# oneapi-src/ishmem

Hardware: AMD Instinct MI355X
Metric: GiB/s device-resident float32 sum-reduce at 1/2/4/8 PEs vs HBM+xGMI roofline (higher is better)
Workload: dtype f32

## Files before the change

include/ishmem_capi.h:

```cpp
#ifndef ISHMEM_AMD_CAPI_H
#define ISHMEM_AMD_CAPI_H

#include <stddef.h>
#include <stdint.h>

#ifdef __cplusplus
extern "C" {
#endif

typedef enum {
    ISHMEMI_OP_AND = 0,
    ISHMEMI_OP_OR = 1,
    ISHMEMI_OP_XOR = 2,
    ISHMEMI_OP_MAX = 3,
    ISHMEMI_OP_MIN = 4,
    ISHMEMI_OP_SUM = 5,
    ISHMEMI_OP_PROD = 6,
    ISHMEMI_OP_COUNT = 7
} ishmemi_c_op_t;

typedef enum {
    ISHMEMI_DT_INT8 = 0,
    ISHMEMI_DT_INT16 = 1,
    ISHMEMI_DT_INT32 = 2,
// ... 99 lines not shown
int ishmemi_c_fence(void);
int ishmemi_c_quiet_on_stream(void *stream);
int ishmemi_c_read_all_u32(void *out, const void *p, size_t n, int grid, void *stream);

#define ISHMEMI_C_MAX_PES 16
#define ISHMEMI_C_MAX_TEAMS 64
#define ISHMEMI_C_DEV_PHASES 4
typedef struct {
    int32_t pe, npes;
    uint64_t timeout_ticks;
    char *heap_base;
    uint64_t heap_size;
    char *peer_heap[ISHMEMI_C_MAX_PES];
    uint32_t *my_dflags;
    uint32_t *peer_dflags[ISHMEMI_C_MAX_PES];
    uint32_t *epochs;
    uint32_t *err;
    int32_t team_start[ISHMEMI_C_MAX_TEAMS], team_stride[ISHMEMI_C_MAX_TEAMS];
    int32_t team_size[ISHMEMI_C_MAX_TEAMS], team_my_idx[ISHMEMI_C_MAX_TEAMS];
    uint64_t *dev_counts;
} ishmemi_c_device_ctx_t;
void *ishmemi_c_device_ctx(void);
int ishmemi_c_register_device_ctx_slot(const void *host_shadow);

const char *ishmemi_c_last_error(void);
int ishmemi_c_set_param(const char *name, long long value);
long long ishmemi_c_get_param(const char *name);
int ishmemi_c_phase_times(float *ms5);
int ishmemi_c_error_count(void);
size_t ishmemi_c_dtype_size(int dtype);
int ishmemi_c_op_dtype_valid(int op, int dtype);
int ishmemi_c_chunk_bounds(uint64_t nitems, int npes, int c, uint64_t *begin, uint64_t *end);
int ishmemi_c_path_limits(int npes, int colocated, long long *ll_limit, long long *fold_limit);
int ishmemi_c_bootstrap_selftest(int pe, int npes, const char *key, int value, int *out);
const char *ishmemi_c_version(void);

#ifdef __cplusplus
}
#endif

#endif
```

ishmem_amd/_lib.py:

```python
from __future__ import annotations

import ctypes
import os
from pathlib import Path

LIB_PATH = Path(__file__).resolve().parent / "libishmem_amd.so"
_VARIANT = os.environ.get("ISHMEM_AMD_LIB")

_vp, _i, _sz, _ll, _u64 = ctypes.c_void_p, ctypes.c_int, ctypes.c_size_t, ctypes.c_longlong, ctypes.c_uint64
PROTOTYPES = [
    ("ishmemi_c_init", _i, []),
    ("ishmemi_c_init_pe", _i, [_i, _i, _i, ctypes.c_char_p]),
    ("ishmemi_c_launch_info", _i, [ctypes.POINTER(_i), ctypes.POINTER(_i), ctypes.POINTER(_i), ctypes.c_char_p, _sz,
                                   ctypes.c_char_p, _sz]),
    ("ishmemi_c_finalize", _i, []),
    ("ishmemi_c_initialized", _i, []),
    ("ishmemi_c_my_pe", _i, []),
    ("ishmemi_c_n_pes", _i, []),
    ("ishmemi_c_device", _i, []),
    ("ishmemi_c_init_thread", _i, [_i, ctypes.POINTER(_i)]),
    ("ishmemi_c_query_thread", _i, [ctypes.POINTER(_i)]),
    ("ishmemi_c_malloc", _vp, [_sz]),
    ("ishmemi_c_align", _vp, [_sz, _sz]),
    ("ishmemi_c_calloc", _vp, [_sz, _sz]),
# ... 23 lines not shown
    ("ishmemi_c_fcollect", _i, [_i, _vp, _vp, _sz]),
    ("ishmemi_c_fcollect_on_stream", _i, [_i, _vp, _vp, _sz, _vp, _vp]),
    ("ishmemi_c_alltoall", _i, [_i, _vp, _vp, _sz]),
    ("ishmemi_c_alltoall_on_stream", _i, [_i, _vp, _vp, _sz, _vp, _vp]),
    ("ishmemi_c_collect_on_stream", _i, [_i, _vp, _vp, _sz, _vp, _vp]),
    ("ishmemi_c_put", _i, [_vp, _vp, _sz, _i]),
    ("ishmemi_c_get", _i, [_vp, _vp, _sz, _i]),
    ("ishmemi_c_put_nbi", _i, [_vp, _vp, _sz, _i]),
    ("ishmemi_c_get_nbi", _i, [_vp, _vp, _sz, _i]),
    ("ishmemi_c_put_on_stream", _i, [_vp, _vp, _sz, _i, _vp]),
    ("ishmemi_c_get_on_stream", _i, [_vp, _vp, _sz, _i, _vp]),
    ("ishmemi_c_quiet", _i, []),
    ("ishmemi_c_fence", _i, []),
    ("ishmemi_c_quiet_on_stream", _i, [_vp]),
    ("ishmemi_c_read_all_u32", _i, [_vp, _vp, _sz, _i, _vp]),
    ("ishmemi_c_stream_wait_events", _i, [_vp, _vp, _sz]),
    ("ishmemi_c_stream_record_event", _i, [_vp, _vp]),
    ("ishmemi_c_collect", _i, [_i, _vp, _vp, _sz]),
    ("ishmemi_c_scan", _i, [_i, _i, _i, _vp, _vp, _sz]),
    ("ishmemi_c_scan_on_stream", _i, [_i, _i, _i, _vp, _vp, _sz, _vp, _vp]),
    ("ishmemi_c_broadcast", _i, [_i, _vp, _vp, _sz, _i]),
    ("ishmemi_c_broadcast_on_stream", _i, [_i, _vp, _vp, _sz, _i, _vp, _vp]),
    ("ishmemi_c_device_ctx", _vp, []),
    ("ishmemi_c_register_device_ctx_slot", _i, [_vp]),
    ("ishmemi_c_last_error", ctypes.c_char_p, []),
    ("ishmemi_c_set_param", _i, [ctypes.c_char_p, _ll]),
    ("ishmemi_c_get_param", _ll, [ctypes.c_char_p]),
    ("ishmemi_c_phase_times", _i, [ctypes.POINTER(ctypes.c_float)]),
    ("ishmemi_c_error_count", _i, []),
    ("ishmemi_c_dtype_size", _sz, [_i]),
    ("ishmemi_c_op_dtype_valid", _i, [_i, _i]),
    ("ishmemi_c_chunk_bounds", _i, [_u64, _i, _i, ctypes.POINTER(_u64), ctypes.POINTER(_u64)]),
    ("ishmemi_c_path_limits", _i, [_i, _i, ctypes.POINTER(_ll), ctypes.POINTER(_ll)]),
    ("ishmemi_c_bootstrap_selftest", _i, [_i, _i, ctypes.c_char_p, _i, ctypes.POINTER(_i)]),
    ("ishmemi_c_version", ctypes.c_char_p, []),
]

_lib = None


def load(build_if_missing: bool = True) -> ctypes.CDLL:
    global _lib
    if _lib is not None:
        return _lib
    if _VARIANT:
        lib = ctypes.CDLL(str(Path(_VARIANT).resolve()), mode=ctypes.RTLD_GLOBAL)
        for name, res, args in PROTOTYPES:
            fn = getattr(lib, name)
            fn.restype = res
            fn.argtypes = args
        _lib = lib
        return lib
    if build_if_missing:
        from . import _build
        if _build.needs_build():
            try:
                _build.build()
            except RuntimeError:
                if not LIB_PATH.exists():
                    raise
    if not LIB_PATH.exists():
        raise ImportError(f"ishmem_amd native library missing: {LIB_PATH} (run __graft_entry__.build())")
    lib = ctypes.CDLL(str(LIB_PATH), mode=ctypes.RTLD_GLOBAL)
    for name, res, args in PROTOTYPES:
        fn = getattr(lib, name)
        fn.restype = res
        fn.argtypes = args
    _lib = lib
    _warn_foreign_runtime()
    return lib


def _warn_foreign_runtime() -> None:
    try:
        with open("/proc/self/maps") as f:
            foreign = any("amdhip64" in line and "/torch/lib/" in line for line in f)
    except OSError:
        return
    if foreign:
        import sys
        print("[ishmem_amd] WARN: the HIP runtime in use is torch's bundled copy (torch was imported "
# ... 3 lines not shown
```

ishmem_amd/csrc/kernels.h:

```cpp
#pragma once
#include <hip/hip_runtime.h>
#include <stddef.h>
#include <stdint.h>

#include "types.h"

namespace ishmemi {

constexpr int kMaxPes = 16;
constexpr int kMaxBlocks = 1024;
constexpr int kPhases = 4;
constexpr int kPhaseStart = 0, kPhaseMid = 1, kPhaseEnd = 2, kPhaseSync = 3;
constexpr size_t kFlagWordsPerTeam = (size_t) kPhases * kMaxBlocks * kMaxPes;
constexpr size_t kTeamFlagBytes = kFlagWordsPerTeam * 4 + 256;
constexpr int kBlock = 256;
constexpr int kUnroll = 4;
constexpr int kFaninBlock = 64;
constexpr int kFaninMaxGrid = (int) ((1ull << 31) / kFaninBlock);

constexpr int kEpWords = 16;
constexpr int kLineWords = 16;
constexpr int kEpReplicas = 64;
constexpr int kEpRepLine = 1, kEpShardLine = kEpRepLine + kEpReplicas, kEpShards = 8;
constexpr int kEpTopLine = kEpShardLine + kEpShards;
// ... 109 lines not shown
constexpr int kRealignMaxGrid = (int) ((1ull << 31) / kRealignBlock);
#ifndef ISHMEMI_RS_REALIGN_BLOCK
#define ISHMEMI_RS_REALIGN_BLOCK 64
#endif
constexpr int kRsRealignBlock = ISHMEMI_RS_REALIGN_BLOCK;
#ifndef ISHMEMI_REALIGN_PEEL
#define ISHMEMI_REALIGN_PEEL 256
#endif
constexpr uint64_t kRealignPeel = ISHMEMI_REALIGN_PEEL;

struct FaninArgs {
    const char *src[kMaxFanin];
    char *dst;
    uint64_t head, nitems, tail;
    int nsrc;
    int realign;
    uint32_t shift[kMaxFanin];
    uint64_t total;
};

struct PhaseArgs {
    const char *src[kMaxPes];
    const char *dstp[kMaxPes];
    char *dst;
    uint64_t head, nitems, tail;
    uint64_t items_per_chunk;
    uint32_t elem;
    int p, me;
    int peer_nt;
    uint32_t shift;
    uint64_t total;
    int whole;
    int xcd_group;
};
hipError_t launch_rs_phase(int op, int dt, const PhaseArgs &a, hipStream_t s);
hipError_t launch_ag_phase(const PhaseArgs &a, hipStream_t s);

hipError_t launch_allreduce(int op, int dt, bool vec, const ReduceArgs &a, int grid,
                            hipStream_t s);
hipError_t launch_fanin(int op, int dt, bool vec, const FaninArgs &a, int grid, hipStream_t s);
hipError_t launch_team_sync(const ReduceArgs &a, hipStream_t s);
hipError_t launch_pull_probe(const FaninArgs &a, int policy, hipStream_t s);
void set_device_share(int share);
int device_share();
constexpr int kWaitSlotsDefault = 16;
void set_wait_slots(int slots);
int wait_slots();
void set_realign_grid_cap(int cap);
int realign_grid_cap();
void set_collect_realign(int on);
int collect_realign();
void set_phase_unaligned(int on);
int phase_unaligned();
hipError_t launch_occupy(int grid, uint64_t usec, hipStream_t s);
hipError_t launch_produce_u32(uint32_t *dst, const uint32_t *a, const uint32_t *b, uint64_t n, hipStream_t s);

struct RmaArgs {
    char *dst;
    const char *src;
    uint64_t head, nitems, tail;
};
hipError_t launch_rma_copy(const RmaArgs &a, bool put, int max_blocks, hipStream_t s);
hipError_t launch_read_all_u32(uint32_t *out, const uint32_t *p, uint64_t n, int grid, hipStream_t s);

}
```

ishmem_amd/csrc/kernels.hip:

```cpp
#include "kernels_impl.h"

namespace ishmemi {

namespace {
int g_device_share = 1;
int g_wait_slots = kWaitSlotsDefault;
}
void set_device_share(int share) { g_device_share = share < 1 ? 1 : share; }
int device_share() { return g_device_share; }
void set_wait_slots(int slots) { g_wait_slots = slots < 1 ? 1 : slots; }
int wait_slots() { return g_wait_slots; }
int g_realign_grid_cap = 0;
void set_realign_grid_cap(int cap) { g_realign_grid_cap = cap < 0 ? 0 : cap; }
int realign_grid_cap() { return g_realign_grid_cap; }
int g_collect_realign = 1;
void set_collect_realign(int on) { g_collect_realign = on != 0; }
int collect_realign() { return g_collect_realign; }
int g_phase_unaligned = 1;
void set_phase_unaligned(int on) { g_phase_unaligned = on != 0; }
int phase_unaligned() { return g_phase_unaligned; }

#define ISHMEMI_DECL_OP(N)                                                                         \
    hipError_t launch_allreduce_op##N(int dt, bool vec, const ReduceArgs &a, int grid,             \
                                      hipStream_t s);                                              \
    hipError_t launch_fanin_op##N(int dt, bool vec, const FaninArgs &a, int grid, hipStream_t s); \
    hipError_t launch_ll_op##N(int dt, const LLArgs &a, hipStream_t s);                            \
    hipError_t launch_rs_phase_op##N(int dt, const PhaseArgs &a, hipStream_t s);
ISHMEMI_DECL_OP(0)
ISHMEMI_DECL_OP(1)
ISHMEMI_DECL_OP(2)
ISHMEMI_DECL_OP(3)
ISHMEMI_DECL_OP(4)
ISHMEMI_DECL_OP(5)
ISHMEMI_DECL_OP(6)

hipError_t launch_allreduce(int op, int dt, bool vec, const ReduceArgs &a, int grid, hipStream_t s)
{
    if (!op_dtype_valid(op, dt)) return hipErrorInvalidValue;
    switch (op) {
        case 0: return launch_allreduce_op0(dt, vec, a, grid, s);
        case 1: return launch_allreduce_op1(dt, vec, a, grid, s);
        case 2: return launch_allreduce_op2(dt, vec, a, grid, s);
        case 3: return launch_allreduce_op3(dt, vec, a, grid, s);
        case 4: return launch_allreduce_op4(dt, vec, a, grid, s);
        case 5: return launch_allreduce_op5(dt, vec, a, grid, s);
        case 6: return launch_allreduce_op6(dt, vec, a, grid, s);
        default: return hipErrorInvalidValue;
// ... 64 lines not shown
```

ishmem_amd/csrc/kernels_impl.h:

```cpp
#pragma once
#include <algorithm>
#include <map>
#include <mutex>
#include <type_traits>

#include "kernels.h"

namespace ishmemi {
namespace {

constexpr int kSysCoherent = 17;
constexpr int kNonTemporal = 2;
constexpr uint64_t kTile = (uint64_t) kBlock * kUnroll;
#ifndef ISHMEMI_AR_OCC
#define ISHMEMI_AR_OCC 4
#endif


template <typename T>
struct alignas(16) Vec {
    T e[16 / sizeof(T)];
};

template <typename T>
// ... 786 lines not shown
    if (i0 + tid < a.nitems) wt_store(make_rsrc(uniform_ptr(a.dst + wo)), tid * 16u, acc);
}

template <typename T, int OP, int NS>
__global__ __launch_bounds__(kRealignBlock) void fanin_realign_kernel(FaninArgs a)
{
    static_assert(NS == 1 || NS == 2, "realigned fan-in: 1 or 2 sources");
    __shared__ u32x4 edge[NS][kRealignWaves + 1];
    const uint32_t tid = threadIdx.x;
    const uint64_t stride = (uint64_t) gridDim.x * kRealignBlock;
    const uint64_t first = (uint64_t) blockIdx.x * kRealignBlock;
    if (stride >= a.nitems) {
        if (first < a.nitems) fanin_realign_block<T, OP, NS>(a, edge, first);
    } else {
        for (uint64_t i0 = first; i0 < a.nitems; i0 += stride) {
            fanin_realign_block<T, OP, NS>(a, edge, i0);
            __syncthreads();
        }
    }
    if (blockIdx.x == 0) {
        const uint64_t tail_off = a.head + a.nitems * (16 / sizeof(T));
        for (int pass = 0; pass < 2; ++pass) {
            const uint64_t cnt = pass == 0 ? a.head : a.tail;
            for (uint64_t t = tid; t < cnt; t += kRealignBlock) {
                const uint64_t e = pass == 0 ? t : tail_off + t;
                T acc = ((const T *) a.src[0])[e];
                if constexpr (NS == 2) acc = op1<T, OP>(acc, ((const T *) a.src[1])[e]);
                ((T *) a.dst)[e] = acc;
            }
        }
    }
}

template <typename T, int OP, int P, bool NT, int R>
__device__ __forceinline__ void rs_phase_item(const PhaseArgs &a, uint64_t wb, bool valid)
{
    using Item = Vec<T>;
    const uint32_t off = threadIdx.x * 16u;
    Item x[P];
#pragma unroll
    for (int k = 0; k < P; ++k) {
        const int j = (R + k) % P;
        if (!valid) continue;
        if (NT || j == a.me) x[k] = bload<Item>(make_rsrc(uniform_ptr(a.src[j] + wb)), off);
        else x[k] = cload<Item>(make_rsrc(uniform_ptr(a.src[j] + wb)), off);
    }
    Item acc = x[(P - R) % P];
#pragma unroll
    for (int j = 1; j < P; ++j) acc = op1<T, OP>(acc, x[(j - R + P) % P]);
    if (valid) wt_store(make_rsrc(uniform_ptr(a.dst + wb)), off, acc);
}

template <typename T, int OP, int P, bool NT, int R = 0>
__device__ __forceinline__ void rs_phase_dispatch(const PhaseArgs &a, int rot, uint64_t wb, bool valid)
{
    if constexpr (R == P - 1) {
        rs_phase_item<T, OP, P, NT, R>(a, wb, valid);
    } else {
        if (rot == R) rs_phase_item<T, OP, P, NT, R>(a, wb, valid);
        else rs_phase_dispatch<T, OP, P, NT, R + 1>(a, rot, wb, valid);
    }
}

template <typename T, int OP>
__device__ __forceinline__ void rs_phase_item_any(const PhaseArgs &a, uint64_t wb, bool valid)
{
    using Item = Vec<T>;
    if (!valid) return;
    const uint32_t off = threadIdx.x * 16u;
    Item acc;
    for (int j = 0; j < a.p; ++j) {
        Item x;
        if (j == a.me || a.peer_nt) x = nt_load((const Item *) (a.src[j] + wb + off));
        else x = cload<Item>(make_rsrc(uniform_ptr(a.src[j] + wb)), off);
        acc = j == 0 ? x : op1<T, OP>(acc, x);
    }
    wt_store(make_rsrc(uniform_ptr(a.dst + wb)), off, acc);
}

template <typename T, int OP>
__device__ __forceinline__ void rs_phase_edges(const PhaseArgs &a)
{
    const int p = a.p, me = a.me;
    if (blockIdx.x == 0) {
        const int tid = threadIdx.x;
        const uint64_t tail_off = a.head + a.nitems * (16 / sizeof(T));
        for (int region = 0; region < 2; ++region) {
            const bool owner = a.whole || (region == 0 ? me == 0 : me == p - 1);
            const uint64_t cnt = region == 0 ? a.head : a.tail;
            if (!owner || (uint64_t) tid >= cnt) continue;
            const uint64_t rbase = (region == 0 ? 0 : tail_off) * sizeof(T);
            const uint32_t off = (uint32_t) (tid * sizeof(T));
            T acc = T();
            for (int j = 0; j < p; ++j) {
                T x;
                if (j == me) x = ((const T *) (a.src[j] + rbase))[tid];
                else x = cload<T>(make_rsrc(uniform_ptr(a.src[j] + rbase)), off);
                acc = (j == 0) ? x : op1<T, OP>(acc, x);
            }
            wt_store(make_rsrc(uniform_ptr(a.dst + rbase)), off, acc);
        }
    }
}

__device__ __forceinline__ uint64_t xcd_grouped_block(uint64_t b, uint64_t grid)
{
    if (b >= (grid & ~63ull)) return b;
    return (b & ~63ull) | ((b & 7) << 3) | ((b >> 3) & 7);
}

template <typename T, int OP, int P>
__global__ __launch_bounds__(kFaninBlock) void rs_phase_kernel(PhaseArgs a)
{
    const int me = a.me;
    const uint64_t cs = a.whole ? 0 : min((uint64_t) me * a.items_per_chunk, a.nitems);
    const uint64_t ce = a.whole ? a.nitems : min(cs + a.items_per_chunk, a.nitems);
    const uint64_t head_bytes = a.head * sizeof(T);
    const uint64_t stride = (uint64_t) gridDim.x * kFaninBlock;
    const uint64_t blk = a.shift && a.xcd_group ? xcd_grouped_block(blockIdx.x, gridDim.x) : blockIdx.x;
    auto body = [&](auto nt) {
        for (uint64_t i0 = cs + blk * kFaninBlock; i0 < ce; i0 += stride) {
            const bool valid = i0 + threadIdx.x < ce;
            const uint64_t wb = head_bytes + i0 * 16;
            if constexpr (P > 0) rs_phase_dispatch<T, OP, P, decltype(nt)::value>(a, (int) ((i0 / kFaninBlock) % P), wb, valid);
            else rs_phase_item_any<T, OP>(a, wb, valid);
        }
    };
    if (a.peer_nt) {
        body(std::true_type{});
    } else {
        body(std::false_type{});
    }
    rs_phase_edges<T, OP>(a);
// ... 62 lines not shown
        const uint64_t je = min(js + a.items_per_chunk, a.nitems);
        const uint64_t i0 = js + (w / peers) * kFaninBlock;
        if (i0 + threadIdx.x < je) {
            const uint64_t wb = head_bytes + i0 * 16;
            const u32x4 x = a.peer_nt ? nt_load((const u32x4 *) (a.dstp[j] + wb + off))
                                      : cload<u32x4>(make_rsrc(uniform_ptr(a.dstp[j] + wb)), off);
            wt_store(make_rsrc(uniform_ptr(a.dst + wb)), off, x);
        }
    }
    if (blockIdx.x == 0) {
        const uint32_t tid = threadIdx.x;
        const uint64_t tail_b = (uint64_t) a.tail * a.elem;
        const uint64_t tail_base = head_bytes + a.nitems * 16;
        if (me != 0 && tid < head_bytes)
            a.dst[tid] = (char) cload<uint8_t>(make_rsrc(uniform_ptr(a.dstp[0])), tid);
        if (me != p - 1 && tid < tail_b)
            a.dst[tail_base + tid] = (char) cload<uint8_t>(make_rsrc(uniform_ptr(a.dstp[p - 1] + tail_base)), tid);
    }
}

template <typename K>
int phase_grid(K, uint64_t items)
{
    const uint64_t g = (items + kFaninBlock - 1) / kFaninBlock;
    return (int) std::max<uint64_t>(1, std::min<uint64_t>(g, (uint64_t) kFaninMaxGrid));
}

template <typename T, int OP>
hipError_t rs_phase_t(const PhaseArgs &a, hipStream_t s)
{
    const uint64_t cs = a.whole ? 0 : std::min((uint64_t) a.me * a.items_per_chunk, a.nitems);
    const uint64_t len = a.whole ? a.nitems : std::min(cs + a.items_per_chunk, a.nitems) - cs;
    auto go = [&](auto kernel) {
        hipLaunchKernelGGL(kernel, dim3(phase_grid(kernel, len)), dim3(kFaninBlock), 0, s, a);
    };
    if (a.shift && !phase_unaligned()) {
        uint64_t g = std::max<uint64_t>(1, std::min<uint64_t>((len + kRsRealignBlock - 1) / kRsRealignBlock,
                                                              (1ull << 31) / kRsRealignBlock));
        if (realign_grid_cap() > 0) g = std::min<uint64_t>(g, (uint64_t) realign_grid_cap());
        hipLaunchKernelGGL((rs_phase_realign_kernel<T, OP>), dim3((unsigned) g), dim3(kRsRealignBlock), 0, s, a);
    } else if (a.p == 2) go(rs_phase_kernel<T, OP, 2>);
    else if (a.p == 4) go(rs_phase_kernel<T, OP, 4>);
    else if (a.p == 8) go(rs_phase_kernel<T, OP, 8>);
    else go(rs_phase_kernel<T, OP, 0>);
    return hipGetLastError();
}

template <typename T, int OP>
__device__ __forceinline__ uint64_t fold8(uint64_t acc, uint64_t x)
{
    constexpr int K = 8 / sizeof(T);
    struct alignas(8) W {
        T e[K];
    };
    W a = __builtin_bit_cast(W, acc), b = __builtin_bit_cast(W, x);
#pragma unroll
    for (int i = 0; i < K; ++i) a.e[i] = op1<T, OP>(a.e[i], b.e[i]);
    return __builtin_bit_cast(uint64_t, a);
}

__device__ __forceinline__ uint64_t ll_load(const char *p, uint64_t valid)
{
    if (valid == 8) {
        if (((uintptr_t) p & 7) == 0) return *(const uint64_t *) p;
        if (((uintptr_t) p & 3) == 0)
            return (uint64_t) ((const uint32_t *) p)[0] | ((uint64_t) ((const uint32_t *) p)[1] << 32);
    }
// ... 230 lines not shown
```

ishmem_amd/csrc/runtime.cpp:

```cpp
#include <hip/hip_runtime.h>
#include <stdio.h>
#include <stdlib.h>
#include <string.h>
#include <strings.h>
#include <stdint.h>
#include <errno.h>
#include <sys/prctl.h>
#include <unistd.h>

#include <algorithm>
#include <chrono>
#include <limits>
#include <map>
#include <mutex>
#include <string>
#include <vector>

#include "bootstrap.h"
#include "kernels.h"
#include "types.h"

namespace ishmemi {
namespace {

// ... 134 lines not shown
    const char *b = s;
    while (*b == ' ' || *b == '\t') ++b;
    char *end = nullptr;
    errno = 0;
    const long long v = strtoll(b, &end, 10);
    const char *e = end;
    while (*e == ' ' || *e == '\t') ++e;
    if (end == b || *e || errno == ERANGE) {
        if (strncmp(name, "ISHMEM_", 7) == 0 && g_env_error.empty())
            g_env_error = std::string(name) + "='" + s + "' is not an integer";
        return dflt;
    }
    return v;
}

bool env_flag_false(const char *name)
{
    const char *s = getenv(name);
    return s && *s && (strcmp(s, "0") == 0 || strcasecmp(s, "false") == 0);
}
bool env_flag_true(const char *name)
{
    const char *s = getenv(name);
    return s && *s && !env_flag_false(name);
}

void warn_unknown_env()
{
    static const char *const known[] = {
        "DEBUG", "ENABLE_VERBOSE_PRINT", "STACK_PRINT_LIMIT", "ENABLE_GPU_IPC", "ENABLE_GPU_IPC_PIDFD",
        "SYMMETRIC_SIZE", "ENABLE_ACCESSIBLE_HOST_HEAP", "NBI_COUNT", "MWAIT_BURST", "SHMEM_LIB_NAME",
        "MPI_LIB_NAME", "PMI_LIB_NAME", "TEAMS_MAX", "TEAM_SHARED_ONLY_SELF", "RUNTIME", "RUNTIME_USE_OSHMPI", "ROOT",
        "PE", "NPES", "DEVICE", "BOOTSTRAP_KEY", "TIMEOUT_MS", "MAX_BLOCKS", "WAIT_SLOTS", "LL_MAX_BYTES",
        "ONESHOT_P2_MAX_BYTES", "PHASED_MIN_BYTES", "PHASED_PEER_NT", "STAGING_SIZE", "STAGING_SLOTS",
        "STAGED_COPY_KERNEL", "STREAM_ORDER", "FLAGS_KIND", "EP_UNCACHED", "BARRIER_KIND", "XGMI_LL_MAX_BYTES",
        "XGMI_FOLD_MAX_BYTES", "TEST_FLAGS_UNAVAILABLE", "TEST_PCI_BUS",
        "AMD_LIB", "OFFLOAD_ARCH", "BENCH_SAME_DEVICE", "BENCH_EMULATE_SHARE1", "BENCH_SETUP_WATCHDOG_S"};
    for (char **e = ::environ; e && *e; ++e) {
        if (strncmp(*e, "ISHMEM_", 7) != 0) continue;
        const char *name = *e + 7, *eq = strchr(name, '=');
        const size_t len = eq ? (size_t) (eq - name) : strlen(name);
        bool ok = false;
        for (const char *k : known) ok = ok || (strlen(k) == len && strncmp(k, name, len) == 0);
        if (!ok) fprintf(stderr, "[ishmem_amd] WARN: Environment variable 'ISHMEM_%.*s' is not a supported variable\n", (int) len, name);
    }
}

long long wait_slots_floor() { return std::max<long long>(1, env_ll("GPU_MAX_HW_QUEUES", 4)); }

struct Team {
    bool valid = false;
    int start = 0, stride = 1, size = 1;
    int my_idx = -1;
    int num_contexts = 0;
    bool colocated = true;
};

struct TeamMem {
    uint32_t *flags[kMaxPes] = {};
    uint64_t *ring[kMaxPes] = {};
    int pool_idx = -1;
    char *fold_scratch = nullptr;
    size_t fold_scratch_bytes = 0;
};

struct PoolBlock {
    uint32_t *ptr = nullptr;
    hipIpcMemHandle_t handle{};
    bool in_use = false;
};

constexpr long long kPhasedOff = std::numeric_limits<long long>::max();
constexpr long long kPhasedDefault = 4ll << 20;

struct PeRecord {
    int32_t pe, pid, device, flags_kind;
    int32_t flags_kind_requested;
    char pci_bus[32];
    uint64_t heap_size;
    int64_t max_blocks, ll_max_bytes, oneshot_p2, phased_min;
    uint64_t staging_bytes;
    int64_t staging_slots;
    int64_t xgmi_ll_max, xgmi_fold_max;
    hipIpcMemHandle_t heap_handle;
    hipIpcMemHandle_t flags_handle;
};

struct State {
    std::mutex mu;
    bool initialized = false;
    int pe = 0, npes = 1, device = 0;
    ShmBootstrap boot;

    char *heap = nullptr;
    size_t heap_size = 0;
    std::map<size_t, size_t> free_list;
    std::map<size_t, size_t> used;
    char *peer_heap[kMaxPes] = {};

    uint32_t *flags = nullptr;
    int flags_kind = 0;
    uint32_t *peer_flags[kMaxPes] = {};
    int dev_id[kMaxPes] = {};
    TeamMem tmem[kMaxTeams];
    int teams_max = kTeamsMaxDefault;
    size_t team_block_bytes = 0;
    std::vector<PoolBlock> team_pool;
    std::map<std::pair<int, uint32_t>, void *> peer_pool;
    uint32_t *err_host = nullptr;
    uint32_t *err_dev = nullptr;
    uint64_t *exch_host = nullptr, *exch_dev = nullptr;
    uint32_t *done_host = nullptr, *done_dev = nullptr;
    uint32_t done_seq = 0;
    int block_spin = 2;
    ishmemi_c_device_ctx_t *dctx = nullptr;
    uint32_t *dev_epochs = nullptr;
    uint32_t *kern_ep = nullptr;

    char *team_scratch = nullptr;
    char *count_slots = nullptr;
    char *staging = nullptr;
    size_t staging_bytes = 0;
    hipStream_t copy_in = nullptr, copy_out = nullptr;
    hipStream_t rma_stream = nullptr;
    hipEvent_t rma_ev = nullptr;
    bool rma_pending = false;
    hipStream_t last_stream = nullptr;
    bool last_stream_set = false;
    bool stream_order = false;
    long long oneshot_p2 = 32ll << 20;
    long long phased_min = kPhasedDefault;
    hipEvent_t order_ev = nullptr;
    hipEvent_t staging_ev = nullptr;
    bool staging_used = false;
    int staging_slots = kStagingSlotsDefault;
    int staged_copy_kernel = 0;
    bool test_flags_unavailable = false;
    int phased_peer_nt = 0;
    int ar_shifted = 1;
    int rs_xcd = 1;
    int direct_p2 = 1;
    int direct_max_pes = 4;
    int direct_inplace = 1;
    long long xgmi_ll_max = -1, xgmi_fold_max = -1;
    double xgmi_link_bps = 76.8e9;
    hipEvent_t ev_in[kMaxStagingSlots] = {}, ev_red[kMaxStagingSlots] = {}, ev_out[kMaxStagingSlots] = {};

    Team teams[kMaxTeams];
    int max_blocks = kMaxBlocks;
    long long ll_max_bytes = (long long) kLLDefaultBytes;
    long long timeout_ms = 60000;
    int debug = 0;
    int error_count = 0;
    uint64_t *trace = nullptr;
    bool phase_events = false, phase_recorded = false;
    hipEvent_t phase_ev[6] = {};
    double init_us[8] = {};
};

const char *const kInitPhase[8] = {"hip", "heap", "flags", "bootstrap", "ipc_heap", "ipc_flags", "teams", "total"};

State &S()
{
    static State s;
    return s;
}

struct CtxSlots {
    std::mutex mu;
    std::vector<const void *> shadows;
};
// ... 244 lines not shown
    if (f.a_us > g.a_us) return 0;
    if (f.b_us_per_byte <= g.b_us_per_byte) return kUnlimited;
    return (long long) ((g.a_us - f.a_us) / (f.b_us_per_byte - g.b_us_per_byte));
}

struct PathLimits {
    long long ll, fold, oneshot;
};

PathLimits path_limits(const State &s, int p, bool colocated)
{
    PathLimits r{0, 0, 0};
    if (p < 2) return r;
    const long long cap = std::min<long long>(std::max<long long>(s.ll_max_bytes, 0), (long long) ll_capacity(p));
    const bool fold_team = s.direct_p2 && p <= s.direct_max_pes;
    if (colocated) {
        r.ll = cap;
        if (p >= 3 && fold_team) r.ll = std::min<long long>(r.ll, (768ll << 10) / p);
        r.fold = p == 2 ? s.oneshot_p2 : s.oneshot_p2 / 4 / (p - 1);
    } else {
        const double L = s.xgmi_link_bps;
        long long ll = crossover(model_ll(p, L), model_rsag(p, L));
        if (fold_team) ll = std::min(ll, crossover(model_ll(p, L), model_fold(p, L)));
        if (s.xgmi_ll_max >= 0) ll = s.xgmi_ll_max;
        r.ll = std::min(cap, ll);
        r.fold = s.xgmi_fold_max >= 0 ? s.xgmi_fold_max : crossover(model_fold(p, L), model_rsag(p, L));
    }
    r.oneshot = r.fold;
    if (!fold_team) r.fold = 0;
    return r;
}

PathLimits team_limits(const State &s, const Team &t) { return path_limits(s, t.size, t.colocated); }

bool ll_eligible(const State &s, const Team &t, const void *dst, const void *src, size_t bytes)
{
    (void) dst;
    (void) src;
    return t.size > 1 && bytes > 0 && (long long) bytes <= team_limits(s, t).ll;
}

bool capturing(hipStream_t st)
{
    hipStreamCaptureStatus cs = hipStreamCaptureStatusNone;
    if (hipStreamIsCapturing(st, &cs) != hipSuccess) {
        (void) hipGetLastError();
        return false;
    }
    return cs != hipStreamCaptureStatusNone;
}

int host_wait(State &s, hipStream_t st)
{
    if (s.block_spin && s.done_dev && !capturing(st)) {
        const uint32_t seq = ++s.done_seq;
        if (hipStreamWriteValue32(st, s.done_dev, seq, 0) == hipSuccess) {
            const auto t0 = std::chrono::steady_clock::now();
            int spins = 0;
            while (__atomic_load_n(s.done_host, __ATOMIC_ACQUIRE) != seq) {
                __builtin_ia32_pause();
                if (++spins == 4096) {
                    spins = 0;
                    if (std::chrono::steady_clock::now() - t0 > std::chrono::milliseconds(20)) break;
                }
            }
            if (s.block_spin == 2 && __atomic_load_n(s.done_host, __ATOMIC_ACQUIRE) == seq) return 0;
// ... 112 lines not shown
        a.tail = pl.tail;
        a.items_per_chunk = pl.items_per_chunk;
        a.seg_items = pl.seg_items;
    }
    const bool disjoint = d0 + nb <= s0 || s0 + nb <= d0;
    const PathLimits lim = team_limits(s, t);
    const bool fold_size = lim.fold > 0 && (long long) nb <= lim.fold;
    char *scratch = nullptr;
    if (fold_size && d0 == s0 && pl.vec && s.direct_inplace && (uint64_t) t.size * nb <= kInplaceFoldBytes) {
        const TeamMem &m = s.tmem[team];
        if (!m.fold_scratch || m.fold_scratch_bytes < nb + 16)
            return fail("reduce: the team's in-place fold scratch is missing");
        scratch = m.fold_scratch + (d0 & 15);
    }
    const bool inplace_fold = scratch != nullptr;
    const bool direct = (fold_size && disjoint && (pl.vec || realign)) || inplace_fold;
    if ((pl.vec || realign) && (direct || (long long) nb >= s.phased_min)) {
        PhaseArgs ph;
        memset(&ph, 0, sizeof(ph));
        for (int j = 0; j < t.size; ++j) {
            ph.src[j] = a.src[j];
            ph.dstp[j] = a.dstp[j];
        }
        ph.dst = a.dst;
        ph.head = pl.head;
        ph.nitems = pl.nitems;
        ph.tail = pl.tail;
        ph.items_per_chunk = pl.items_per_chunk;
        ph.elem = (uint32_t) es;
        ph.p = t.size;
        ph.me = t.my_idx;
        ph.peer_nt = s.phased_peer_nt;
        ph.whole = direct ? 1 : 0;
        ph.xcd_group = s.rs_xcd && device_share() == 1 ? 1 : 0;
        if (inplace_fold) ph.dst = scratch;
        if (realign) {
            const uint64_t h = std::min<uint64_t>(n, ((16 - d0 % 16) % 16) / es);
            ph.head = h;
            ph.nitems = (n - h) * es / 16;
            ph.tail = n - h - ph.nitems * (16 / es);
            ph.items_per_chunk = items_per_chunk(ph.nitems, t.size);
            ph.shift = (uint32_t) ((s0 + h * es) % 16);
            ph.total = nb;
        }
        const bool ev = s.phase_events && !capturing(st);
        auto mark = [&](int k) -> int {
            if (ev) HIP_TRY(hipEventRecord(s.phase_ev[k], st));
            return 0;
        };
        if (mark(0)) return 1;
        if (team_barrier(s, team, a, st)) return 1;
        if (mark(1)) return 1;
        HIP_TRY(launch_rs_phase(op, dt, ph, st));
        if (mark(2)) return 1;
        if (!direct) {
            if (team_barrier(s, team, a, st)) return 1;
            if (mark(3)) return 1;
            HIP_TRY(launch_ag_phase(ph, st));
        } else if (mark(3)) {
            return 1;
        }
        if (mark(4)) return 1;
        if (team_barrier(s, team, a, st)) return 1;
        if (mark(5)) return 1;
        if (inplace_fold && launch_copy(dst, scratch, nb, st)) return 1;
        s.phase_recorded = s.phase_recorded || ev;
        return 0;
    }
    if (t.size == 2 && (long long) nb <= lim.oneshot && disjoint) {
        a.oneshot = 1;
        a.items_per_chunk = pl.nitems;
        a.seg_items = seg_items(pl.nitems);
        pl.grid = (int) std::max<uint64_t>(
            1, std::min<uint64_t>(nsegs(pl.nitems, a.seg_items), (uint64_t) s.max_blocks));
    }
    HIP_TRY(launch_allreduce(op, dt, pl.vec, a, pl.grid, st));
    return 0;
}

constexpr size_t kPinMinBytes = (size_t) 1 << 20;

bool pageable_host(const void *p)
{
    hipPointerAttribute_t attr;
    if (hipPointerGetAttributes(&attr, p) != hipSuccess) {
        (void) hipGetLastError();
        return true;
    }
// ... 746 lines not shown
    if (env_flag_false("ISHMEM_ENABLE_GPU_IPC") && g_env_error.empty())
        g_env_error = std::string("ISHMEM_ENABLE_GPU_IPC=") + getenv("ISHMEM_ENABLE_GPU_IPC") +
                      " is not supported: ishmem_amd's collectives are IPC-only (peer loads over xGMI from "
                      "IPC-mapped heaps; there is no proxy path)";
    if (env_flag_true("ISHMEM_ENABLE_ACCESSIBLE_HOST_HEAP") && g_env_error.empty())
        g_env_error = std::string("ISHMEM_ENABLE_ACCESSIBLE_HOST_HEAP=") + getenv("ISHMEM_ENABLE_ACCESSIBLE_HOST_HEAP") +
                      " is not supported: the symmetric heap is device memory shared over IPC (host buffers "
                      "are accepted by every call and staged)";
    s.max_blocks = (int) std::min<long long>(kMaxBlocks, std::max<long long>(1, env_ll("ISHMEM_MAX_BLOCKS", kMaxBlocks)));
    s.timeout_ms = std::max<long long>(1, env_ll("ISHMEM_TIMEOUT_MS", 60000));
    s.ll_max_bytes = std::min<long long>((long long) kLLMaxBytes,
                                         std::max<long long>(0, env_bytes("ISHMEM_LL_MAX_BYTES", (long long) kLLDefaultBytes)));
    s.debug = debug_level();
    s.trace = nullptr;
    s.stream_order = env_ll("ISHMEM_STREAM_ORDER", 0) != 0;
    s.oneshot_p2 = std::max<long long>(0, env_bytes("ISHMEM_ONESHOT_P2_MAX_BYTES", 32ll << 20));
    s.phased_min = env_bytes("ISHMEM_PHASED_MIN_BYTES", kPhasedDefault);
    if (s.phased_min < 0) s.phased_min = kPhasedOff;
    s.staging_bytes = (env_size("ISHMEM_STAGING_SIZE", (size_t) 128 << 20) + kHeapAlign - 1) &
                      ~(size_t) (kHeapAlign - 1);
    s.staging_slots = (int) std::min<long long>(kMaxStagingSlots, std::max<long long>(2, env_ll("ISHMEM_STAGING_SLOTS", kStagingSlotsDefault)));
    s.staged_copy_kernel = (int) (env_ll("ISHMEM_STAGED_COPY_KERNEL", kStagedCopyKernelDefault) & 3);
    const size_t heap_request = env_size("ISHMEM_SYMMETRIC_SIZE", (size_t) 4 << 30);
    const int first_kind = (int) std::min<long long>(kFlagsCoarse, std::max<long long>(0, env_ll("ISHMEM_FLAGS_KIND", 0)));
#ifdef ISHMEMI_TEST_HOOKS
    s.test_flags_unavailable = env_ll("ISHMEM_TEST_FLAGS_UNAVAILABLE", 0) != 0;
#else
    for (const char *hook : {"ISHMEM_TEST_FLAGS_UNAVAILABLE", "ISHMEM_TEST_PCI_BUS"})
        if (getenv(hook) && g_env_error.empty())
            g_env_error = std::string(hook) + " is a test hook, honoured only by libishmem_amd_testhooks.so";
#endif
    const bool ep_uncached = env_ll("ISHMEM_EP_UNCACHED", 0) != 0;
    s.phased_peer_nt = env_ll("ISHMEM_PHASED_PEER_NT", 0) != 0;
    s.teams_max = kTeamsMaxDefault;
    if (const char *tm = getenv("ISHMEM_TEAMS_MAX"); tm && *tm) {
        const long long v = env_ll("ISHMEM_TEAMS_MAX", kTeamsMaxDefault);
        if (v < 0 && g_env_error.empty())
            g_env_error = std::string("ISHMEM_TEAMS_MAX='") + tm + "' is not a team count";
        else if (v > kMaxTeams && g_env_error.empty())
            g_env_error = "ISHMEM_TEAMS_MAX=" + std::to_string(v) + ": requested " + std::to_string(v) +
                          " teams, but only " + std::to_string(kMaxTeams) + " are supported";
        s.teams_max = (int) std::min<long long>(kMaxTeams, std::max<long long>(kPredefTeams, v));
    }
    s.xgmi_ll_max = std::max<long long>(-1, env_bytes("ISHMEM_XGMI_LL_MAX_BYTES", -1));
    s.xgmi_fold_max = std::max<long long>(-1, env_bytes("ISHMEM_XGMI_FOLD_MAX_BYTES", -1));
    s.xgmi_link_bps = 76.8e9;
    if (const char *bk = getenv("ISHMEM_BARRIER_KIND"); bk && *bk && strcasecmp(bk, "kernel") != 0 && g_env_error.empty())
        g_env_error = std::string("ISHMEM_BARRIER_KIND='") + bk +
                      "' is not supported: team barriers are the one-workgroup barrier kernel ('kernel')";
    if (!g_env_error.empty()) {
        const std::string e = g_env_error;
        g_env_error.clear();
        return fail("init: " + e);
    }
    warn_unknown_env();

    using clk = std::chrono::steady_clock;
    const auto t_start = clk::now();
    auto t_mark = t_start;
    auto phase_done = [&](int k) {
        const auto now = clk::now();
        s.init_us[k] = std::chrono::duration<double, std::micro>(now - t_mark).count();
        t_mark = now;
        if (s.debug > 1) {
            fprintf(stderr, "[ishmem_amd] PE %d init: %s done (%.1f ms)\n", pe, kInitPhase[k], s.init_us[k] / 1000.0);
            fflush(stderr);
// ... 36 lines not shown

    for (int i = 0; i < kMaxPes; ++i) {
        s.peer_heap[i] = nullptr;
        s.peer_flags[i] = nullptr;
    }
    s.peer_heap[pe] = s.heap;
    s.peer_flags[pe] = s.flags;
    for (int i = 0; i < kMaxPes; ++i) s.dev_id[i] = 0;
    phase_done(2);

    if (npes > 1) {
        struct PtracerWindow {
            PtracerWindow() { prctl(PR_SET_PTRACER, PR_SET_PTRACER_ANY, 0, 0, 0); }
            ~PtracerWindow() { prctl(PR_SET_PTRACER, 0, 0, 0, 0); }
        } ptracer_window;
        std::string err;
        if (s.boot.attach(pe, npes, key, (int) std::max<long long>(s.timeout_ms, 10000), err))
            return fail(err);
        PeRecord mine{};
        mine.pe = pe;
        mine.pid = (int32_t) getpid();
        mine.device = s.device;
        mine.flags_kind = s.flags_kind;
        mine.flags_kind_requested = first_kind;
        mine.heap_size = s.heap_size;
        mine.max_blocks = s.max_blocks;
        mine.ll_max_bytes = s.ll_max_bytes;
        mine.oneshot_p2 = s.oneshot_p2;
        mine.phased_min = s.phased_min;
        mine.staging_bytes = s.staging_bytes;
        mine.staging_slots = s.staging_slots;
        mine.xgmi_ll_max = s.xgmi_ll_max;
        mine.xgmi_fold_max = s.xgmi_fold_max;
        if (hipDeviceGetPCIBusId(mine.pci_bus, sizeof(mine.pci_bus), s.device) != hipSuccess) {
            (void) hipGetLastError();
            snprintf(mine.pci_bus, sizeof(mine.pci_bus), "dev%d", s.device);
        }
#ifdef ISHMEMI_TEST_HOOKS
        if (const char *fake = getenv("ISHMEM_TEST_PCI_BUS"))
            snprintf(mine.pci_bus, sizeof(mine.pci_bus), "%s", fake);
#endif
        if (hipError_t e = hipIpcGetMemHandle(&mine.heap_handle, s.heap); e != hipSuccess)
            return fail(std::string("init: hipIpcGetMemHandle of the symmetric heap: ") + hipGetErrorString(e) + ipc_hint());
        mine.flags_handle = flags_handle;
        PeRecord all[kMaxPes];
        if (s.boot.allgather(&mine, all, sizeof(PeRecord), err)) return fail(err);
        phase_done(3);
        for (int j = 0; j < npes; ++j) {
            s.ll_max_bytes = std::min<long long>(s.ll_max_bytes, all[j].ll_max_bytes);
            s.oneshot_p2 = std::min<long long>(s.oneshot_p2, all[j].oneshot_p2);
            s.phased_min = std::max<long long>(s.phased_min, all[j].phased_min);
            s.staging_bytes = std::min<size_t>(s.staging_bytes, all[j].staging_bytes);
            s.staging_slots = (int) std::min<int64_t>(s.staging_slots, all[j].staging_slots);
            if (all[j].xgmi_ll_max >= 0)
                s.xgmi_ll_max = s.xgmi_ll_max < 0 ? all[j].xgmi_ll_max : std::min<long long>(s.xgmi_ll_max, all[j].xgmi_ll_max);
            if (all[j].xgmi_fold_max >= 0)
                s.xgmi_fold_max = s.xgmi_fold_max < 0 ? all[j].xgmi_fold_max
                                                       : std::min<long long>(s.xgmi_fold_max, all[j].xgmi_fold_max);
        }
        int share = 0;
        for (int j = 0; j < npes; ++j)
            share += strncmp(all[j].pci_bus, mine.pci_bus, sizeof(mine.pci_bus)) == 0;
        for (int j = 0; j < npes; ++j) {
            s.dev_id[j] = j;
            for (int k = 0; k < j; ++k)
                if (strncmp(all[j].pci_bus, all[k].pci_bus, sizeof(all[j].pci_bus)) == 0) {
                    s.dev_id[j] = s.dev_id[k];
                    break;
                }
        }
        bool coarse_forced = false;
        for (int j = 0; j < npes; ++j) coarse_forced = coarse_forced || all[j].flags_kind_requested == kFlagsCoarse;
        set_device_share(share);
        for (int j = 0; j < npes; ++j) {
            if (j == pe) continue;
            if (all[j].heap_size != s.heap_size)
                return fail("init: ISHMEM_SYMMETRIC_SIZE differs between PEs");
            if (all[j].device != s.device) {
                int can = 0;
                if (hipDeviceCanAccessPeer(&can, s.device, all[j].device) != hipSuccess || !can)
                    return fail("init: no peer access from device " + std::to_string(s.device) +
                                " to device " + std::to_string(all[j].device) + " (PE " +
                                std::to_string(j) + ")");
                hipError_t e = hipDeviceEnablePeerAccess(all[j].device, 0);
                if (e != hipSuccess && e != hipErrorPeerAccessAlreadyEnabled)
                    return hipfail("hipDeviceEnablePeerAccess", e);
                (void) hipGetLastError();
            }
            if (hipError_t e = hipIpcOpenMemHandle((void **) &s.peer_heap[j], all[j].heap_handle,
                                                   hipIpcMemLazyEnablePeerAccess);
                e != hipSuccess)
// ... 1202 lines not shown

const char *ishmemi_c_last_error(void) { return g_last_error.c_str(); }

int ishmemi_c_phase_times(float *ms5)
{
    State &s = S();
    if (!ms5) return fail("phase_times: null output");
    if (!s.phase_recorded || !s.phase_ev[0]) return fail("phase_times: no phased reduce recorded (set_param phase_events 1)");
    HIP_TRY(hipEventSynchronize(s.phase_ev[5]));
    for (int k = 0; k < 5; ++k) HIP_TRY(hipEventElapsedTime(&ms5[k], s.phase_ev[k], s.phase_ev[k + 1]));
    return 0;
}

int ishmemi_c_set_param(const char *name, long long value)
{
    State &s = S();
    std::lock_guard<std::mutex> lk(s.mu);
    const std::string n = name ? name : "";
    if (n == "max_blocks") s.max_blocks = (int) std::min<long long>(kMaxBlocks, std::max<long long>(1, value));
    else if (n == "staged_copy_kernel") s.staged_copy_kernel = (int) (value & 3);
    else if (n == "wait_slots") {
        if (value < wait_slots_floor())
            return fail("set_param: wait_slots " + std::to_string(value) + " is below " +
                        std::to_string(wait_slots_floor()) + " (GPU_MAX_HW_QUEUES), see ISHMEM_WAIT_SLOTS");
        set_wait_slots((int) std::min<long long>(1 << 20, value));
    }
    else if (n == "timeout_ms") s.timeout_ms = std::max<long long>(1, value);
    else if (n == "stream_order") s.stream_order = value != 0;
    else if (n == "oneshot_p2_max_bytes") s.oneshot_p2 = std::max<long long>(0, value);
    else if (n == "phased_min_bytes") s.phased_min = value < 0 ? kPhasedOff : value;
    else if (n == "ll_max_bytes") s.ll_max_bytes = std::min<long long>((long long) kLLMaxBytes, std::max<long long>(0, value));
    else if (n == "debug") s.debug = (int) value;
    else if (n == "phased_peer_nt") s.phased_peer_nt = value != 0;
    else if (n == "xgmi_ll_max_bytes") s.xgmi_ll_max = std::max<long long>(-1, value);
    else if (n == "xgmi_fold_max_bytes") s.xgmi_fold_max = std::max<long long>(-1, value);
    else if (n == "xgmi_link_mbps") {
        if (value <= 0) return fail("set_param: xgmi_link_mbps must be positive");
        s.xgmi_link_bps = (double) value * 1e6;
    }
    else if (n == "realign_grid_cap") set_realign_grid_cap((int) std::min<long long>(std::max<long long>(value, 0), 1 << 30));
    else if (n == "collect_realign") set_collect_realign((int) (value != 0));
    else if (n == "ar_shifted") s.ar_shifted = value != 0;
    else if (n == "rs_xcd") s.rs_xcd = value != 0;
    else if (n == "direct_p2") s.direct_p2 = value != 0;
    else if (n == "direct_inplace") s.direct_inplace = value != 0;
    else if (n == "block_spin") s.block_spin = (int) std::min<long long>(std::max<long long>(value, 0), 2);
    else if (n == "direct_max_pes") s.direct_max_pes = (int) std::min<long long>(std::max<long long>(value, 2), kMaxPes);
    else if (n == "phase_unaligned") set_phase_unaligned((int) (value != 0));
    else if (n == "trace_buffer") s.trace = (uint64_t *) (uintptr_t) value;
    else if (n == "phase_events") {
        if (value && !s.phase_ev[0])
            for (hipEvent_t &e : s.phase_ev) HIP_TRY(hipEventCreate(&e));
        s.phase_events = value != 0;
    }
    else return fail("set_param: unknown parameter " + n);
    return 0;
}

long long ishmemi_c_get_param(const char *name)
{
    State &s = S();
    const std::string n = name ? name : "";
    if (n == "max_blocks") return s.max_blocks;
    if (n == "staged_copy_kernel") return s.staged_copy_kernel;
    if (n == "wait_slots") return wait_slots();
    if (n == "timeout_ms") return s.timeout_ms;
    if (n == "stream_order") return s.stream_order ? 1 : 0;
    if (n == "oneshot_p2_max_bytes") return s.oneshot_p2;
    if (n == "phased_min_bytes") return s.phased_min == kPhasedOff ? -1 : s.phased_min;
    if (n == "ll_max_bytes") return s.ll_max_bytes;
    if (n == "ll_capacity_bytes") return (long long) ll_capacity(s.npes);
    if (n == "ll_limit_bytes") return team_limits(s, s.teams[0]).ll;
    if (n == "fold_limit_bytes") return team_limits(s, s.teams[0]).fold;
    if (n == "team_colocated") return s.teams[0].colocated ? 1 : 0;
    if (n == "xgmi_ll_max_bytes") return s.xgmi_ll_max;
    if (n == "xgmi_fold_max_bytes") return s.xgmi_fold_max;
    if (n == "xgmi_link_mbps") return (long long) (s.xgmi_link_bps / 1e6);
    if (n == "teams_max") return s.teams_max;
    if (n == "flag_block_bytes") return s.initialized ? (long long) (kBaseAllocBytes + s.team_block_bytes) : 0;
    if (n == "flag_block_pool_bytes") return (long long) (s.team_pool.size() * kTeamAllocBytes);
    if (n == "flag_block_bytes_round5") return (long long) kRound5FlagBytes;
    for (int k = 0; k < 8; ++k)
        if (n == std::string("init_us_") + kInitPhase[k]) return (long long) s.init_us[k];
    if (n == "debug") return s.debug;
    if (n == "phased_peer_nt") return s.phased_peer_nt;
    if (n == "realign_grid_cap") return realign_grid_cap();
    if (n == "collect_realign") return collect_realign();
    if (n == "ar_shifted") return s.ar_shifted;
    if (n == "rs_xcd") return s.rs_xcd;
    if (n == "direct_p2") return s.direct_p2;
    if (n == "direct_inplace") return s.direct_inplace;
    if (n == "block_spin") return s.block_spin;
    if (n == "direct_max_pes") return s.direct_max_pes;
    if (n == "phase_unaligned") return phase_unaligned();
    if (n == "flags_fine_grained") return s.flags_kind != kFlagsCoarse ? 1 : 0;
    if (n == "flags_kind") return s.flags_kind;
    if (n == "staging_bytes") return (long long) s.staging_bytes;
    if (n == "staging_slots") return s.staging_slots;
    if (n == "heap_bytes") return (long long) s.heap_size;
    if (n == "device_share") return device_share();
    if (n == "launch_words") return (long long) (uintptr_t) s.kern_ep;
    if (n == "cu_count") {
        int dev = 0, cus = 0;
        if (hipGetDevice(&dev) != hipSuccess ||
            hipDeviceGetAttribute(&cus, hipDeviceAttributeMultiprocessorCount, dev) != hipSuccess) {
            (void) hipGetLastError();
            return -1;
        }
        return cus;
    }
    return -1;
}

int ishmemi_c_error_count(void)
{
    State &s = S();
    int pending = 0;
    if (s.err_host)
        for (int t = 0; t <= kMaxTeams; ++t)
            pending += __atomic_load_n(&s.err_host[t], __ATOMIC_ACQUIRE) != 0;
    return s.error_count + pending;
}

size_t ishmemi_c_dtype_size(int dtype)
{
    return (dtype >= 0 && dtype < ISHMEMI_DT_COUNT) ? dtype_size(dtype) : 0;
}

int ishmemi_c_op_dtype_valid(int op, int dtype) { return op_dtype_valid(op, dtype) ? 1 : 0; }

int ishmemi_c_chunk_bounds(uint64_t nitems, int npes, int c, uint64_t *begin, uint64_t *end)
{
    if (npes < 1 || c < 0 || c >= npes || !begin || !end) return 1;
    const uint64_t ipc = npes > 1 ? items_per_chunk(nitems, npes) : nitems;
    *begin = std::min<uint64_t>((uint64_t) c * ipc, nitems);
    *end = std::min<uint64_t>(*begin + ipc, nitems);
    return 0;
}

int ishmemi_c_path_limits(int npes, int colocated, long long *ll_limit, long long *fold_limit)
{
    if (npes < 1 || npes > kMaxPes || !ll_limit || !fold_limit) return fail("path_limits: invalid arguments");
    State &s = S();
    std::lock_guard<std::mutex> lk(s.mu);
    const PathLimits r = path_limits(s, npes, colocated != 0);
    *ll_limit = r.ll;
    *fold_limit = r.fold;
    return 0;
}

int ishmemi_c_bootstrap_selftest(int pe, int npes, const char *key, int value, int *out)
{
    ShmBootstrap b;
    std::string err;
    if (b.attach(pe, npes, key ? key : "selftest", 20000, err)) return fail(err);
    if (b.allgather(&value, out, sizeof(int), err)) return fail(err);
    if (b.barrier(err)) return fail(err);
    return 0;
}

const char *ishmemi_c_version(void) { return "ishmem_amd 0.1.0 (reduction path; ref ishmem 1.5.1)"; }

}
```

Baseline: 3142.

## Push reduced chunks to all peers in reduce-scatter phase, skipping allgather

Adds a push mode to the phased reduce path. After each PE reduces its chunk, it writes the result directly to every peer's destination, with a rotated peer order to spread link traffic. This removes the team barrier and the separate allgather phase. It is enabled by default for colocated teams, and the setting is agreed across PEs at init. It also adds a tunable grid cap for the phase kernel. The cost is extra remote write traffic issued from the reduce kernel, and completion now depends on ordering assumptions that the dropped barrier used to enforce.

```diff
diff --git a/include/ishmem_capi.h b/include/ishmem_capi.h
--- a/include/ishmem_capi.h
+++ b/include/ishmem_capi.h
@@ -155,6 +155,7 @@
 int ishmemi_c_op_dtype_valid(int op, int dtype);
 int ishmemi_c_chunk_bounds(uint64_t nitems, int npes, int c, uint64_t *begin, uint64_t *end);
 int ishmemi_c_path_limits(int npes, int colocated, long long *ll_limit, long long *fold_limit);
+int ishmemi_c_phased_push_resolve(const long long *per_pe, int npes, int colocated);
 int ishmemi_c_bootstrap_selftest(int pe, int npes, const char *key, int value, int *out);
 const char *ishmemi_c_version(void);
 
diff --git a/ishmem_amd/_lib.py b/ishmem_amd/_lib.py
--- a/ishmem_amd/_lib.py
+++ b/ishmem_amd/_lib.py
@@ -79,6 +79,7 @@
     ("ishmemi_c_op_dtype_valid", _i, [_i, _i]),
     ("ishmemi_c_chunk_bounds", _i, [_u64, _i, _i, ctypes.POINTER(_u64), ctypes.POINTER(_u64)]),
     ("ishmemi_c_path_limits", _i, [_i, _i, ctypes.POINTER(_ll), ctypes.POINTER(_ll)]),
+    ("ishmemi_c_phased_push_resolve", _i, [ctypes.POINTER(_ll), _i, _i]),
     ("ishmemi_c_bootstrap_selftest", _i, [_i, _i, ctypes.c_char_p, _i, ctypes.POINTER(_i)]),
     ("ishmemi_c_version", ctypes.c_char_p, []),
 ]
@@ -93,7 +94,9 @@
     if _VARIANT:
         lib = ctypes.CDLL(str(Path(_VARIANT).resolve()), mode=ctypes.RTLD_GLOBAL)
         for name, res, args in PROTOTYPES:
-            fn = getattr(lib, name)
+            fn = getattr(lib, name, None)
+            if fn is None:
+                continue
             fn.restype = res
             fn.argtypes = args
         _lib = lib
diff --git a/ishmem_amd/csrc/kernels.h b/ishmem_amd/csrc/kernels.h
--- a/ishmem_amd/csrc/kernels.h
+++ b/ishmem_amd/csrc/kernels.h
@@ -165,6 +165,7 @@
     uint64_t total;
     int whole;
     int xcd_group;
+    int push;
 };
 hipError_t launch_rs_phase(int op, int dt, const PhaseArgs &a, hipStream_t s);
 hipError_t launch_ag_phase(const PhaseArgs &a, hipStream_t s);
@@ -181,6 +182,8 @@
 int wait_slots();
 void set_realign_grid_cap(int cap);
 int realign_grid_cap();
+void set_phase_grid_cap(int cap);
+int phase_grid_cap();
 void set_collect_realign(int on);
 int collect_realign();
 void set_phase_unaligned(int on);
diff --git a/ishmem_amd/csrc/kernels.hip b/ishmem_amd/csrc/kernels.hip
--- a/ishmem_amd/csrc/kernels.hip
+++ b/ishmem_amd/csrc/kernels.hip
@@ -13,6 +13,9 @@
 int g_realign_grid_cap = 0;
 void set_realign_grid_cap(int cap) { g_realign_grid_cap = cap < 0 ? 0 : cap; }
 int realign_grid_cap() { return g_realign_grid_cap; }
+int g_phase_grid_cap = 0;
+void set_phase_grid_cap(int cap) { g_phase_grid_cap = cap < 0 ? 0 : cap; }
+int phase_grid_cap() { return g_phase_grid_cap; }
 int g_collect_realign = 1;
 void set_collect_realign(int on) { g_collect_realign = on != 0; }
 int collect_realign() { return g_collect_realign; }
diff --git a/ishmem_amd/csrc/kernels_impl.h b/ishmem_amd/csrc/kernels_impl.h
--- a/ishmem_amd/csrc/kernels_impl.h
+++ b/ishmem_amd/csrc/kernels_impl.h
@@ -842,6 +842,23 @@
     }
 }
 
+template <int P, typename Item>
+__device__ __forceinline__ void rs_phase_push(const PhaseArgs &a, int rot, uint64_t wb, uint32_t off, const Item &acc)
+{
+    if constexpr (P > 0) {
+#pragma unroll
+        for (int k = 0; k < P; ++k) {
+            const int j = (rot + k) % P;
+            wt_store(make_rsrc(uniform_ptr((j == a.me ? a.dst : a.dstp[j]) + wb)), off, acc);
+        }
+    } else {
+        for (int k = 0; k < a.p; ++k) {
+            const int j = (rot + k) % a.p;
+            wt_store(make_rsrc(uniform_ptr((j == a.me ? a.dst : a.dstp[j]) + wb)), off, acc);
+        }
+    }
+}
+
 template <typename T, int OP, int P, bool NT, int R>
 __device__ __forceinline__ void rs_phase_item(const PhaseArgs &a, uint64_t wb, bool valid)
 {
@@ -858,7 +875,9 @@
     Item acc = x[(P - R) % P];
 #pragma unroll
     for (int j = 1; j < P; ++j) acc = op1<T, OP>(acc, x[(j - R + P) % P]);
-    if (valid) wt_store(make_rsrc(uniform_ptr(a.dst + wb)), off, acc);
+    if (!valid) return;
+    if (a.push) rs_phase_push<P>(a, R, wb, off, acc);
+    else wt_store(make_rsrc(uniform_ptr(a.dst + wb)), off, acc);
 }
 
 template <typename T, int OP, int P, bool NT, int R = 0>
@@ -885,7 +904,8 @@
         else x = cload<Item>(make_rsrc(uniform_ptr(a.src[j] + wb)), off);
         acc = j == 0 ? x : op1<T, OP>(acc, x);
     }
-    wt_store(make_rsrc(uniform_ptr(a.dst + wb)), off, acc);
+    if (a.push) rs_phase_push<0>(a, (int) ((wb / (kFaninBlock * 16)) % (uint64_t) a.p), wb, off, acc);
+    else wt_store(make_rsrc(uniform_ptr(a.dst + wb)), off, acc);
 }
 
 template <typename T, int OP>
@@ -909,6 +929,9 @@
                 acc = (j == 0) ? x : op1<T, OP>(acc, x);
             }
             wt_store(make_rsrc(uniform_ptr(a.dst + rbase)), off, acc);
+            if (a.push)
+                for (int j = 0; j < p; ++j)
+                    if (j != me) wt_store(make_rsrc(uniform_ptr(a.dstp[j] + rbase)), off, acc);
         }
     }
 }
@@ -1037,7 +1060,9 @@
     const uint64_t cs = a.whole ? 0 : std::min((uint64_t) a.me * a.items_per_chunk, a.nitems);
     const uint64_t len = a.whole ? a.nitems : std::min(cs + a.items_per_chunk, a.nitems) - cs;
     auto go = [&](auto kernel) {
-        hipLaunchKernelGGL(kernel, dim3(phase_grid(kernel, len)), dim3(kFaninBlock), 0, s, a);
+        int g = phase_grid(kernel, len);
+        if (phase_grid_cap() > 0) g = std::min(g, phase_grid_cap());
+        hipLaunchKernelGGL(kernel, dim3(g), dim3(kFaninBlock), 0, s, a);
     };
     if (a.shift && !phase_unaligned()) {
         uint64_t g = std::max<uint64_t>(1, std::min<uint64_t>((len + kRsRealignBlock - 1) / kRsRealignBlock,
diff --git a/ishmem_amd/csrc/runtime.cpp b/ishmem_amd/csrc/runtime.cpp
--- a/ishmem_amd/csrc/runtime.cpp
+++ b/ishmem_amd/csrc/runtime.cpp
@@ -190,7 +190,7 @@
         "SYMMETRIC_SIZE", "ENABLE_ACCESSIBLE_HOST_HEAP", "NBI_COUNT", "MWAIT_BURST", "SHMEM_LIB_NAME",
         "MPI_LIB_NAME", "PMI_LIB_NAME", "TEAMS_MAX", "TEAM_SHARED_ONLY_SELF", "RUNTIME", "RUNTIME_USE_OSHMPI", "ROOT",
         "PE", "NPES", "DEVICE", "BOOTSTRAP_KEY", "TIMEOUT_MS", "MAX_BLOCKS", "WAIT_SLOTS", "LL_MAX_BYTES",
-        "ONESHOT_P2_MAX_BYTES", "PHASED_MIN_BYTES", "PHASED_PEER_NT", "STAGING_SIZE", "STAGING_SLOTS",
+        "ONESHOT_P2_MAX_BYTES", "PHASED_MIN_BYTES", "PHASED_PEER_NT", "PHASED_PUSH","STAGING_SIZE", "STAGING_SLOTS",
         "STAGED_COPY_KERNEL", "STREAM_ORDER", "FLAGS_KIND", "EP_UNCACHED", "BARRIER_KIND", "XGMI_LL_MAX_BYTES",
         "XGMI_FOLD_MAX_BYTES", "TEST_FLAGS_UNAVAILABLE", "TEST_PCI_BUS",
         "AMD_LIB", "OFFLOAD_ARCH", "BENCH_SAME_DEVICE", "BENCH_EMULATE_SHARE1", "BENCH_SETUP_WATCHDOG_S"};
@@ -240,6 +240,7 @@
     uint64_t staging_bytes;
     int64_t staging_slots;
     int64_t xgmi_ll_max, xgmi_fold_max;
+    int64_t phased_push;
     hipIpcMemHandle_t heap_handle;
     hipIpcMemHandle_t flags_handle;
 };
@@ -295,6 +296,7 @@
     int staged_copy_kernel = 0;
     bool test_flags_unavailable = false;
     int phased_peer_nt = 0;
+    int phased_push = -1;
     int ar_shifted = 1;
     int rs_xcd = 1;
     int direct_p2 = 1;
@@ -605,6 +607,16 @@
 }
 
 PathLimits team_limits(const State &s, const Team &t) { return path_limits(s, t.size, t.colocated); }
+
+long long agree_phased_push(const long long *per_pe, int npes)
+{
+    long long v = -1;
+    for (int j = 0; j < npes; ++j)
+        if (per_pe[j] >= 0) v = v < 0 ? std::min<long long>(per_pe[j], 1) : std::min<long long>(v, per_pe[j]);
+    return v;
+}
+
+bool phased_push_on(long long setting, bool colocated) { return setting < 0 ? colocated : setting != 0; }
 
 bool ll_eligible(const State &s, const Team &t, const void *dst, const void *src, size_t bytes)
 {
@@ -783,6 +795,8 @@
         ph.me = t.my_idx;
         ph.peer_nt = s.phased_peer_nt;
         ph.whole = direct ? 1 : 0;
+        const bool push = !direct && pl.vec && (disjoint || d0 == s0) && phased_push_on(s.phased_push, t.colocated);
+        ph.push = push ? 1 : 0;
         ph.xcd_group = s.rs_xcd && device_share() == 1 ? 1 : 0;
         if (inplace_fold) ph.dst = scratch;
         if (realign) {
@@ -804,7 +818,7 @@
         if (mark(1)) return 1;
         HIP_TRY(launch_rs_phase(op, dt, ph, st));
         if (mark(2)) return 1;
-        if (!direct) {
+        if (!direct && !push) {
             if (team_barrier(s, team, a, st)) return 1;
             if (mark(3)) return 1;
             HIP_TRY(launch_ag_phase(ph, st));
@@ -1617,6 +1631,7 @@
 #endif
     const bool ep_uncached = env_ll("ISHMEM_EP_UNCACHED", 0) != 0;
     s.phased_peer_nt = env_ll("ISHMEM_PHASED_PEER_NT", 0) != 0;
+    s.phased_push = (int) std::min<long long>(1, std::max<long long>(-1, env_ll("ISHMEM_PHASED_PUSH", -1)));
     s.teams_max = kTeamsMaxDefault;
     if (const char *tm = getenv("ISHMEM_TEAMS_MAX"); tm && *tm) {
         const long long v = env_ll("ISHMEM_TEAMS_MAX", kTeamsMaxDefault);
@@ -1719,6 +1734,7 @@
         mine.staging_slots = s.staging_slots;
         mine.xgmi_ll_max = s.xgmi_ll_max;
         mine.xgmi_fold_max = s.xgmi_fold_max;
+        mine.phased_push = s.phased_push;
         if (hipDeviceGetPCIBusId(mine.pci_bus, sizeof(mine.pci_bus), s.device) != hipSuccess) {
             (void) hipGetLastError();
             snprintf(mine.pci_bus, sizeof(mine.pci_bus), "dev%d", s.device);
@@ -1744,6 +1760,11 @@
             if (all[j].xgmi_fold_max >= 0)
                 s.xgmi_fold_max = s.xgmi_fold_max < 0 ? all[j].xgmi_fold_max
                                                        : std::min<long long>(s.xgmi_fold_max, all[j].xgmi_fold_max);
+        }
+        {
+            long long push[kMaxPes];
+            for (int j = 0; j < npes; ++j) push[j] = all[j].phased_push;
+            s.phased_push = (int) agree_phased_push(push, npes);
         }
         int share = 0;
         for (int j = 0; j < npes; ++j)
@@ -3012,6 +3033,7 @@
     else if (n == "ll_max_bytes") s.ll_max_bytes = std::min<long long>((long long) kLLMaxBytes, std::max<long long>(0, value));
     else if (n == "debug") s.debug = (int) value;
     else if (n == "phased_peer_nt") s.phased_peer_nt = value != 0;
+    else if (n == "phased_push") s.phased_push = value < 0 ? -1 : value != 0;
     else if (n == "xgmi_ll_max_bytes") s.xgmi_ll_max = std::max<long long>(-1, value);
     else if (n == "xgmi_fold_max_bytes") s.xgmi_fold_max = std::max<long long>(-1, value);
     else if (n == "xgmi_link_mbps") {
@@ -3019,6 +3041,7 @@
         s.xgmi_link_bps = (double) value * 1e6;
     }
     else if (n == "realign_grid_cap") set_realign_grid_cap((int) std::min<long long>(std::max<long long>(value, 0), 1 << 30));
+    else if (n == "phase_grid_cap") set_phase_grid_cap((int) std::min<long long>(std::max<long long>(value, 0), 1 << 30));
     else if (n == "collect_realign") set_collect_realign((int) (value != 0));
     else if (n == "ar_shifted") s.ar_shifted = value != 0;
     else if (n == "rs_xcd") s.rs_xcd = value != 0;
@@ -3064,7 +3087,9 @@
         if (n == std::string("init_us_") + kInitPhase[k]) return (long long) s.init_us[k];
     if (n == "debug") return s.debug;
     if (n == "phased_peer_nt") return s.phased_peer_nt;
+    if (n == "phased_push") return phased_push_on(s.phased_push, s.teams[0].colocated) ? 1 : 0;
     if (n == "realign_grid_cap") return realign_grid_cap();
+    if (n == "phase_grid_cap") return phase_grid_cap();
     if (n == "collect_realign") return collect_realign();
     if (n == "ar_shifted") return s.ar_shifted;
     if (n == "rs_xcd") return s.rs_xcd;
@@ -3118,6 +3143,15 @@
     return 0;
 }
 
+int ishmemi_c_phased_push_resolve(const long long *per_pe, int npes, int colocated)
+{
+    if (!per_pe || npes < 1 || npes > kMaxPes) {
+        (void) fail("phased_push_resolve: invalid arguments");
+        return -1;
+    }
+    return phased_push_on(agree_phased_push(per_pe, npes), colocated != 0) ? 1 : 0;
+}
+
 int ishmemi_c_path_limits(int npes, int colocated, long long *ll_limit, long long *fold_limit)
 {
     if (npes < 1 || npes > kMaxPes || !ll_limit || !fold_limit) return fail("path_limits: invalid arguments");
```

After: 3141. About the same (-0.0%).
